# mozack/vdjer

Measured on AMD Instinct MI355X. Metric: M paired-reads/sec (k-mer build + contig score), IgH 50bp PE, higher is better.
Workload: dtype u8/u64 (2-bit packed bases, integer counts)

## Files before the change

### vdjer_amd/csrc/vdjx_score.hip

```cpp
#include "vdjx_common.h"
#include "vdjx_scan.h"

#include <algorithm>
#include <numeric>
#include <string.h>
#include <stdlib.h>
#include <stdio.h>

#define NONE32 0xFFFFFFFFu

__host__ __device__ inline int base_code(char ch) {
	const unsigned c = (unsigned char) ch;
	const int code = (int) ((0xD8u >> (((c >> 1) & 3u) * 2u)) & 3u);
	return (c == 'A' || c == 'C' || c == 'G' || c == 'T') ? code : -1;
}

extern "C" int vdjx_vregion_load(vdjx_ctx* c, const char* const* lines, size_t n_lines, int vk) {
	if (!c || (n_lines && !lines)) { vdjx_set_error("vdjx_vregion_load: NULL argument"); return VDJX_EINVAL; }
	if (vk < 2 || vk > 16) { vdjx_set_error("vregion k-mer size %d outside [2,16]", vk); return VDJX_ELIMIT; }
	HIP_TRY(hipSetDevice(c->device));
	vdjx_clear_errors();
	std::vector<u32> off(n_lines + 1, 0);
	std::string text;
	for (size_t i = 0; i < n_lines; i++) {
// ... 760 lines not shown
	auto drain = [&]() {
		vdjx_wave_lds_fence();
		for (u32 q0 = 0; q0 < qn; q0 += 64) {
			const u32 qi = q0 + (u32) lane;
			bool pr = false;
			u64 e = 0;
			u32 pos2 = 0, which = 0, o = 0;
			if (qi < qn) {
				e = q_ent[wv][qi]; o = q_off[wv][qi];
				pr = map_eval_entry(L, ix.rl, (int) o, e, pos2, which);
			}
			const u64 m = __ballot(pr);
			if (m) {
				u32 base = 0;
				if (lane == 0) base = atomicAdd(&pair_cnt[wi], (u32) __popcll(m));
				base = (u32) __builtin_amdgcn_readlane((int) base, 0);
				if (pr) {
					const u32 mult = ent_count(e);
					pairs[base + (u32) __popcll(m & ((1ull << lane) - 1ull))] = ((u64) mult << 32) | ((o + 1) << 16) | pos2;
					mine += mult;
				}
			}
		}
		vdjx_wave_lds_fence();
		qn = 0;
	};
	for (;;) {
		u32 hb = 0;
		if (lane == 0) hb = atomicAdd(&s_next, 64u * WP_K);
		hb = (u32) __builtin_amdgcn_readlane((int) hb, 0);
		if (hb >= h1) break;
		int orow = 0;
		{
			const u32 hr = hb + (u32) lane * 64u;
			if (lane < WP_K && hr < h1) {
				int lo = 0, hi = noff;
				while (hi - lo > 1) { const int mid = (lo + hi) >> 1; if (L.hpre[mid] <= hr) lo = mid; else hi = mid; }
				orow = lo;
			}
		}
		u64 ent[WP_K];
		u32 oo[WP_K / 2];
#pragma unroll
		for (int u = 0; u < WP_K; u++) {
			const u32 h = hb + (u32) (u * 64 + lane);
			int o = __builtin_amdgcn_readlane(orow, u);
			u64 e = ~0ull;
			if (h < h1) {
				while (h >= L.hpre[o + 1]) o++;
				e = ix.d8[L.cstart[o] + (h - L.hpre[o])];
			}
			ent[u] = e;
			if (u & 1) oo[u >> 1] |= (u32) o << 16; else oo[u >> 1] = (u32) o;
		}
#pragma unroll
		for (int u = 0; u < WP_K; u++) {
			if (hb + (u32) (u * 64) >= h1) break;
			const bool pass = map_entry_present(L, ent[u]) && hb + (u32) (u * 64 + lane) < h1;
			const u64 m = __ballot(pass);
			if (!m) continue;
			if (pass) {
				const u32 at = qn + (u32) __popcll(m & ((1ull << lane) - 1ull));
				q_ent[wv][at] = ent[u];
				q_off[wv][at] = (unsigned short) ((oo[u >> 1] >> (16 * (u & 1))) & 0xFFFFu);
			}
			qn += (u32) __popcll(m);
			if (qn > WP_Q - 64) drain();
		}
	}
	drain();
	mine = (u32) __builtin_amdgcn_readlane(vdjx_wave_scan_add((int) mine), 63);
	if (lane == 0 && mine) atomicAdd(&pair_np[wi], mine);
}

#define GP_G 8
#ifndef GP_THREADS
#define GP_THREADS 768
#define GP_WAVES 6
#define GP_K 12
#define GP_Q 128
#endif
#define GP_TS 4096u
#define GP_DMAX 2048u
#define GP_NOFF 512
#define GP_OCC (GP_G * GP_NOFF)
#define GP_PRESENT_LOG2 16
#ifndef GP_XCD_TILE
#define GP_XCD_TILE 1
#endif
static_assert(GP_Q >= 128, "a drain of full rows must find one");
struct GroupImg {
	u32 key[GP_TS];
	unsigned short didx[GP_TS];
	u32 hpre[GP_DMAX + 1];
	u32 cstart[GP_DMAX];
	unsigned short occ_start[GP_DMAX + 2];
	unsigned short wmask[GP_DMAX];
	unsigned short occ[GP_OCC];
	u32 present[1u << (GP_PRESENT_LOG2 - 5)];
};
__device__ inline int gp_lookup(const GroupImg& L, u32 cls) {
	u32 slot = cls & (GP_TS - 1);
	for (;;) {
		const u32 cur = L.key[slot];
		if (cur == 0) return -1;
		if (cur == cls + 1) return (int) L.didx[slot];
		slot = (slot + 1) & (GP_TS - 1);
	}
}
__device__ inline u32 gp_present_bit2(u32 cls) { return (cls * 0x9E3779B1u) >> (32 - GP_PRESENT_LOG2); }
__device__ inline bool gp_entry_present(const GroupImg& L, const u64 e) {
	const u32 ca = ent_a(e), cb = ent_b(e);
	const u32 ba = ca & ((1u << GP_PRESENT_LOG2) - 1u), bb = cb & ((1u << GP_PRESENT_LOG2) - 1u);
	const u32 ha = (L.present[ba >> 5] >> (ba & 31)) & 1u, hb = (L.present[bb >> 5] >> (bb & 31)) & 1u;
	if (!(ha | hb)) return false;
	const u32 ba2 = gp_present_bit2(ca), bb2 = gp_present_bit2(cb);
	return ((ha & (L.present[ba2 >> 5] >> (ba2 & 31))) | (hb & (L.present[bb2 >> 5] >> (bb2 & 31)))) & 1u;
}

__global__ __launch_bounds__(GP_THREADS, GP_WAVES) void k_group_pairs(ReadIndexDev ix, const uint4* __restrict__ prep, const u32* __restrict__ hits, u32 n, int len,
                                                              const u32* __restrict__ gorder, const u64* __restrict__ pair_off, u64* __restrict__ pair_buf,
                                                              u32* __restrict__ pair_cnt, u32* __restrict__ pair_np, u32* __restrict__ done, unsigned long long* __restrict__ gstat, u32 dbg_in,
                                                              u64 cap) {
#ifdef VDJX_ABLATE
	const u32 dbg = dbg_in;
#else
	(void) dbg_in;
	constexpr u32 dbg = 0u;
#endif
	if (pair_off[n] + 1 > cap) return;
	const long long t_begin = clock64();
	__shared__ GroupImg L;
	__shared__ u64 q_ent[GP_THREADS / 64][GP_Q];
	__shared__ unsigned short q_d[GP_THREADS / 64][GP_Q];
	__shared__ u64 s_pbase[GP_G];
	__shared__ u32 s_w[GP_G], s_pcnt[GP_G], s_np[GP_G], s_tmp[GP_THREADS / 64];
	__shared__ u32 s_nd, s_next, s_over;
	const int noff = len - ix.rl;
	const u32 tid = threadIdx.x;
	const int lane = __lane_id();
	const u32 wv = tid >> 6;
	u32 gblk = blockIdx.x;
#ifndef GP_XCD_M
#define GP_XCD_M 32u
#endif
	if (GP_XCD_TILE && (gblk | (8u * GP_XCD_M - 1u)) < gridDim.x) gblk = (gblk & ~(8u * GP_XCD_M - 1u)) | ((gblk & 7u) * GP_XCD_M) | ((gblk >> 3) & (GP_XCD_M - 1u));
	if (tid < GP_G) {
		const u32 idx = gblk * GP_G + tid;
		const u32 wi = idx < n ? gorder[idx] : NONE32;
		s_w[tid] = wi;
		s_pbase[tid] = wi != NONE32 ? pair_off[wi] : 0ull;
		s_pcnt[tid] = 0; s_np[tid] = 0;
	}
	if (tid == 0) { s_nd = 0; s_next = 0; s_over = 0; }
	for (u32 i = tid; i < GP_TS; i += GP_THREADS) L.key[i] = 0;
	for (u32 i = tid; i < (1u << (GP_PRESENT_LOG2 - 5)); i += GP_THREADS) L.present[i] = 0;
	__syncthreads();
	if (tid == 0) {
		u64 tot = 0;
		for (int w = 0; w < GP_G; w++) if (s_w[w] != NONE32) tot += hits[s_w[w]];
		if (tot >> 32) s_over = 1;
	}
	const u32 items = (u32) GP_G * (u32) noff;
	for (u32 it = tid; it < items; it += GP_THREADS) {
		const u32 w = it / (u32) noff, o = it - w * (u32) noff;
		if (s_w[w] == NONE32) continue;
		const uint4 p = prep[(size_t) s_w[w] * noff + o];
		const u32 cls = p.x;
		if (cls == NONE32) continue;
		const u32 pb = cls & ((1u << GP_PRESENT_LOG2) - 1u), pb2 = gp_present_bit2(cls);
		atomicOr(&L.present[pb >> 5], 1u << (pb & 31));
		atomicOr(&L.present[pb2 >> 5], 1u << (pb2 & 31));
		u32 slot = cls & (GP_TS - 1);
		for (u32 probes = 0;; probes++) {
			u32 cur = L.key[slot];
			if (cur == 0) {
				cur = atomicCAS(&L.key[slot], 0u, cls + 1);
				if (cur == 0) {
					const u32 d = atomicAdd(&s_nd, 1u);
					if (d < GP_DMAX) { L.didx[slot] = (unsigned short) d; L.cstart[d] = p.y; L.hpre[d] = p.z; }
					else s_over = 1;
					break;
				}
			}
			if (cur == cls + 1) break;
			slot = (slot + 1) & (GP_TS - 1);
			if (probes >= GP_TS) { s_over = 1; break; }
		}
	}
	__syncthreads();
	if (s_over) { if (tid == 0) atomicAdd(&gstat[1], 1ull); return; }
	const u32 nd = s_nd;
	u32* ocnt = (u32*) &q_ent[0][0];
	for (u32 i = tid; i < nd; i += GP_THREADS) ocnt[i] = 0;
	__syncthreads();
	for (u32 it = tid; it < items; it += GP_THREADS) {
		const u32 w = it / (u32) noff, o = it - w * (u32) noff;
		if (s_w[w] == NONE32) continue;
		const u32 cls = prep[(size_t) s_w[w] * noff + o].x;
		if (cls != NONE32) atomicAdd(&ocnt[gp_lookup(L, cls)], 1u);
	}
	__syncthreads();
	{
		constexpr u32 PER = (GP_DMAX + GP_THREADS) / GP_THREADS;
		u32 hv[PER], cv[PER], hs = 0, cs = 0;
#pragma unroll
		for (u32 j = 0; j < PER; j++) {
			const u32 a = PER * tid + j;
			hv[j] = a < nd ? L.hpre[a] : 0u; cv[j] = a < nd ? ocnt[a] : 0u;
			hs += hv[j]; cs += cv[j];
		}
		u32 htot, ctot;
		u32 hx = vdjx_block_scan(hs, s_tmp, htot);
		u32 cx = vdjx_block_scan(cs, s_tmp, ctot);
		__syncthreads();
#pragma unroll
		for (u32 j = 0; j < PER; j++) {
			const u32 a = PER * tid + j;
			if (a <= nd) { L.hpre[a] = hx; L.occ_start[a] = (unsigned short) cx; }
			if (a < nd) ocnt[a] = 0;
			hx += hv[j]; cx += cv[j];
		}
	}
	__syncthreads();
	for (int w = 0; w < GP_G; w++) {
		if (s_w[w] != NONE32)
			for (int o = (int) tid; o < noff; o += GP_THREADS) {
				const u32 cls = prep[(size_t) s_w[w] * noff + o].x;
				if (cls == NONE32) continue;
				const int d = gp_lookup(L, cls);
				L.occ[L.occ_start[d] + (atomicAdd(&ocnt[d], 1u) & 0xFFFFu)] = (unsigned short) ((u32) w << 10 | (u32) o);
				if (atomicOr(&ocnt[d], 0x10000u << w) & (0x10000u << w)) atomicOr(&ocnt[d], 0x80000000u);
			}
		__syncthreads();
	}
	for (u32 i = tid; i < nd; i += GP_THREADS) L.wmask[i] = (unsigned short) (ocnt[i] >> 16);
	__syncthreads();
	const u32 H = dbg == 2 ? 0u : L.hpre[nd];
	if (tid == 0) { atomicAdd(&gstat[0], (unsigned long long) H); atomicAdd(&gstat[2], (unsigned long long) nd); }
	u32 qn = 0, nq = 0;
	auto drain = [&](bool all) {
		vdjx_wave_lds_fence();
		const u32 upto = all ? qn : qn & ~63u;
		for (u32 q0 = 0; q0 < (dbg == 1 ? 0u : upto); q0 += 64) {
			const u32 qi = q0 + (u32) lane;
			if (qi >= qn) continue;
			const u64 e = q_ent[wv][qi];
			const u32 d = q_d[wv][qi];
			const u32 ca = ent_a(e), cb = ent_b(e);
			u32 as = 0, ae = 0, bs = 0, be = 0;
			int xa = -1, xb = -1;
			if (ca != RI_ENT_NONE) { xa = gp_lookup(L, ca); if (xa >= 0) { as = L.occ_start[xa]; ae = L.occ_start[xa + 1]; } }
			if (cb != RI_ENT_NONE) { xb = gp_lookup(L, cb); if (xb >= 0) { bs = L.occ_start[xb]; be = L.occ_start[xb + 1]; } }
			if (as == ae && bs == be) continue;
			const u32 fl = ent_flags(e), mult = ent_count(e);
			const u32 rc1 = (fl & RI_RC) ? 1u : 0u;
			const u32 mc = L.wmask[d], ma = as < ae ? (u32) L.wmask[xa] : 0u, mb = bs < be ? (u32) L.wmask[xb] : 0u;
			const u32 cs = L.occ_start[d];
			auto emit = [&](u32 w, u32 o, u32 la, u32 lb) {
				const u32 which = (lb && lb >= la) ? 1u : 0u;
				const u32 best = which ? lb : la;
				const u32 rc2 = (fl & (which ? RI_RCB : RI_RCA)) ? 1u : 0u;
				if (rc1 == rc2) return;
				const int dd = (int) (o + 1) - (int) best;
				const int insert = (int) (short) ((dd < 0 ? -dd : dd) + ix.rl);
				if (insert < 50 || insert > 400) return;
				const u32 pos = atomicAdd(&s_pcnt[w], 1u);
				pair_buf[s_pbase[w] + pos] = ((u64) mult << 32) | ((o + 1) << 16) | best;
				atomicAdd(&s_np[w], mult);
			};
			if (!((mc | ma | mb) & 0x8000u)) {
				for (u32 m = mc & (ma | mb); m; m &= m - 1) {
					const u32 w = (u32) __ffs((int) m) - 1u, below = (1u << w) - 1u;
					const u32 o = (u32) L.occ[cs + (u32) __popc(mc & below)] & 1023u;
					const u32 la = (ma >> w) & 1u ? ((u32) L.occ[as + (u32) __popc(ma & below)] & 1023u) + 1u : 0u;
					const u32 lb = (mb >> w) & 1u ? ((u32) L.occ[bs + (u32) __popc(mb & below)] & 1023u) + 1u : 0u;
					emit(w, o, la, lb);
				}
				continue;
			}
			u32 i = cs;
			const u32 ce = L.occ_start[d + 1];
			while (i < ce) {
				const u32 w = (u32) L.occ[i] >> 10;
				u32 la = 0, lb = 0;
				while (as < ae && ((u32) L.occ[as] >> 10) < w) as++;
				while (as < ae && ((u32) L.occ[as] >> 10) == w) { const u32 x = ((u32) L.occ[as] & 1023u) + 1u; la = x > la ? x : la; as++; }
				while (bs < be && ((u32) L.occ[bs] >> 10) < w) bs++;
				while (bs < be && ((u32) L.occ[bs] >> 10) == w) { const u32 x = ((u32) L.occ[bs] & 1023u) + 1u; lb = x > lb ? x : lb; bs++; }
				for (; i < ce && ((u32) L.occ[i] >> 10) == w; i++)
					if (la | lb) emit(w, (u32) L.occ[i] & 1023u, la, lb);
			}
		}
		const u32 rem = qn - upto;
		u64 me = 0; unsigned short md = 0;
		if ((u32) lane < rem) { me = q_ent[wv][upto + (u32) lane]; md = q_d[wv][upto + (u32) lane]; }
		vdjx_wave_lds_fence();
		if ((u32) lane < rem && upto) { q_ent[wv][lane] = me; q_d[wv][lane] = md; }
		vdjx_wave_lds_fence();
		qn = rem;
	};
	for (;;) {
		u32 hb = 0;
		if (lane == 0) hb = atomicAdd(&s_next, 64u * GP_K);
		hb = (u32) __builtin_amdgcn_readlane((int) hb, 0);
		if (hb >= H) break;
		int drow = 0;
		{
			const u32 hr = hb + (u32) lane * 64u;
			if (lane < GP_K && hr < H) {
				int lo = 0, hi = (int) nd;
				while (hi - lo > 1) { const int mid = (lo + hi) >> 1; if (L.hpre[mid] <= hr) lo = mid; else hi = mid; }
				drow = lo;
			}
		}
		u64 ent[GP_K];
		u32 dd[GP_K / 2];
#pragma unroll
		for (int u = 0; u < GP_K; u++) {
			const u32 h = hb + (u32) (u * 64 + lane);
			int d = __builtin_amdgcn_readlane(drow, u);
			u64 e = ~0ull;
			if (h < H) {
				while (h >= L.hpre[d + 1]) d++;
				e = ix.d8[L.cstart[d] + (h - L.hpre[d])];
			}
			ent[u] = e;
			if (u & 1) dd[u >> 1] |= (u32) d << 16; else dd[u >> 1] = (u32) d;
		}
#pragma unroll
		for (int u = 0; u < GP_K; u++) {
			if (hb + (u32) (u * 64) >= H) break;
			const bool pass = gp_entry_present(L, ent[u]) && hb + (u32) (u * 64 + lane) < H;
			const u64 m = __ballot(pass);
			if (!m) continue;
			if (pass) {
				const u32 at = qn + (u32) __popcll(m & ((1ull << lane) - 1ull));
				q_ent[wv][at] = ent[u];
				q_d[wv][at] = (unsigned short) ((dd[u >> 1] >> (16 * (u & 1))) & 0xFFFFu);
			}
			qn += (u32) __popcll(m); nq += (u32) __popcll(m);
			if (qn > GP_Q - 64) drain(false);
		}
	}
	drain(true);
	if (lane == 0 && nq) atomicAdd(&gstat[3], (unsigned long long) nq);
	__syncthreads();
	if (tid < GP_G && s_w[tid] != NONE32) { pair_cnt[s_w[tid]] = s_pcnt[tid]; pair_np[s_w[tid]] = s_np[tid]; done[s_w[tid]] = 1u; }
	if (tid == 0) {
		const unsigned long long dt = (unsigned long long) (clock64() - t_begin);
		atomicAdd(&gstat[4], dt);
		atomicMax(&gstat[5], dt);
	}
}

__global__ __launch_bounds__(MAP_THREADS) void k_window_cover(int len, int rl, vdjx_cov_params cp, const u32* __restrict__ order,
                                                              const u64* __restrict__ pair_off, const u64* __restrict__ pair_buf,
                                                              const u32* __restrict__ pair_cnt, uint8_t* __restrict__ out_valid,
                                                              u64* __restrict__ dbg) {
	const long long t_begin = dbg ? clock64() : 0;
	constexpr int HF_WORDS = MAP_MAXOFF + VDJX_MAX_READ_LEN + 2;
	static_assert(4 * ((HF_WORDS + COV_WORDS) * 4 + 3 * 4) <= 160 * 1024, "k_window_cover: 4 workgroups per CU need hf + diff + flags <= 40 KiB");
	__shared__ u32 hf[HF_WORDS];
	__shared__ int diff[COV_WORDS];
	__shared__ u32 s_bad, s_ok;
	__shared__ int s_firstv;
	const u32 tid = threadIdx.x;
	const int D = len + 1;
	const int e0 = cp.eval_start, e1 = cp.eval_stop, fl = cp.floor;
	const int gap = rl - cp.read_span;
	const int clo = cp.insert_low - rl - cp.mate_span / 2;
	const int chi = cp.insert_high - rl + cp.mate_span / 2;
	const int npos = e1 - e0;
	const int stride = npos + 1;
	const int DB = COV_WORDS / stride;
	const u32 wi = order[blockIdx.x];
	const u64* pairs = pair_buf + pair_off[wi];
	const u32 npairs = pair_cnt[wi];
	if (fl == 0) { if (tid == 0) out_valid[wi] = 1; return; }
	const u32 wv = tid >> 6, NW = MAP_THREADS / 64;
	u32* hp = (u32*) diff;
	const bool priv = (u32) (D + 1) * NW <= COV_WORDS;
	for (u32 i = tid; i < (u32) D + 1; i += MAP_THREADS) hf[i] = 0;
	if (priv) for (u32 i = tid; i < (u32) (D + 1) * NW; i += MAP_THREADS) hp[i] = 0;
	if (tid == 0) { s_bad = 0; s_ok = 0; }
	__syncthreads();
	u32* myh = priv ? hp + wv * (u32) (D + 1) : hf;
	for (u32 q = tid; q < npairs; q += MAP_THREADS) {
		const u64 pe = pairs[q];
		const u32 pr = (u32) pe, mult = (u32) (pe >> 32);
		atomicAdd(&myh[pr >> 16], mult);
		atomicAdd(&myh[pr & 0xFFFFu], mult);
	}
	__syncthreads();
	if (priv) {
		for (u32 i = tid; i < (u32) D + 1; i += MAP_THREADS) {
			u32 sum = 0;
			for (u32 w2 = 0; w2 < NW; w2++) sum += hp[w2 * (u32) (D + 1) + i];
			hf[i] = sum;
		}
		__syncthreads();
	}
	if (tid < 64) {
		const int per = (D + 63) / 64;
		const int a0 = (int) tid * per;
		const int b0 = a0 + per < D ? a0 + per : D;
		u32 sum = 0;
		for (int q = a0; q < b0; q++) sum += hf[q];
		const u32 incl = (u32) vdjx_wave_scan_add((int) sum);
		u32 run = incl - sum;
		for (int q = a0; q < b0; q++) { run += hf[q]; hf[q] = run; }
	}
	if (tid == 0) s_firstv = 0x7FFFFFFF;
	__syncthreads();
	{
		const int n_ent = (int) hf[D - 1];
		const int vmax = e1 - cp.read_span + 1;
		const int vlo = e0 > 1 ? e0 : 1;
		for (int v = vlo + (int) tid; v <= vmax && v < D; v += MAP_THREADS) {
			const int cv = (int) hf[v], cv1 = (int) hf[v - 1];
			if (cv == cv1) continue;
			atomicMin(&s_firstv, v);
			const int i0 = cv1;
			if (i0 < fl) s_bad = 1;
			const int pg = v - gap - 1;
// ... 356 lines not shown
	const int noff = len - ix.rl;
	char* d_s;
	u32 *d_hits, *d_inst;
	PlanOut* d_tot;
	HIP_TRY(db.alloc(&d_s, n * len));
	HIP_TRY(db.alloc(&mp->d_prep, n * (size_t) noff));
	HIP_TRY(db.alloc(&d_hits, n));
	HIP_TRY(db.alloc(&d_inst, n));
	HIP_TRY(db.alloc(&mp->d_off, n + 1));
	HIP_TRY(db.alloc(&mp->d_order, n));
	HIP_TRY(db.alloc(&mp->d_wstart, n + 1));
	HIP_TRY(db.alloc(&d_tot, 1));
	u64 *d_gkey = nullptr, *d_gkey2 = nullptr;
	u32* d_gidx = nullptr;
	if (grouped) {
		HIP_TRY(db.alloc(&d_gkey, n));
		HIP_TRY(db.alloc(&d_gkey2, n));
		HIP_TRY(db.alloc(&d_gidx, n));
		HIP_TRY(db.alloc(&mp->d_gorder, n));
	}
	mp->d_hits = d_hits;
	const char* d_src = nullptr;
	if (vdjx_host_block_holds(c, strings, n * (size_t) len)) d_src = strings;
	const u32 pieces = d_src ? 1u : n * (size_t) len >= (2u << 20) ? 4u : 1u;
	if (pieces > 1) {
		HIP_TRY(hipEventRecord(c->ev_up[0], st));
		HIP_TRY(hipStreamWaitEvent(c->up_stream, c->ev_up[0], 0));
	}
	for (u32 pc = 0; pc < pieces; pc++) {
		const size_t a = n * (size_t) pc / pieces, b = n * (size_t) (pc + 1) / pieces;
		if (pieces > 1) {
			HIP_TRY(hipMemcpyAsync(d_s + a * len, strings + a * len, (b - a) * len, hipMemcpyHostToDevice, c->up_stream));
			HIP_TRY(hipEventRecord(c->ev_up[1 + pc], c->up_stream));
			HIP_TRY(hipStreamWaitEvent(st, c->ev_up[1 + pc], 0));
		} else if (!d_src)
			HIP_TRY(hipMemcpyAsync(d_s, strings, n * len, hipMemcpyHostToDevice, st));
		vdjx_prof_scope ps(c, "k_map_classify");
		const dim3 grid((u32) std::min<size_t>(b - a, 8192));
		if (d_src) d_s = const_cast<char*>(d_src);
		if (c->ri_pool->W == 2) hipLaunchKernelGGL(k_map_classify<2>, grid, dim3(MAP_THREADS), 0, st, ix, d_s, (u32) b, len, weighted, mp->d_prep, d_hits, d_inst, d_gkey, d_gidx, (u32) a);
		else hipLaunchKernelGGL(k_map_classify<VDJX_LONG_W>, grid, dim3(MAP_THREADS), 0, st, ix, d_s, (u32) b, len, weighted, mp->d_prep, d_hits, d_inst, d_gkey, d_gidx, (u32) a);
	}
	{
		vdjx_prof_scope ps(c, "k_plan");
		const bool staged = n * 4 <= 96 * 1024;
		if (staged) HIP_TRY(hipFuncSetAttribute((const void*) k_plan, hipFuncAttributeMaxDynamicSharedMemorySize, 96 * 1024));
		hipLaunchKernelGGL(k_plan, dim3(1), dim3(1024), staged ? n * 4 : 0, st, d_hits, d_inst, (u32) n, chunk_fixed, weighted ? 1 : 0, weighted ? 1 : 0, mp->d_off, mp->d_order, mp->d_wstart, d_tot,
		                   staged ? 1 : 0);
	}
	if (grouped) {
		vdjx_prof_scope ps(c, "group_sort");
		const int rc = vdjx_sort_pairs(db, st, d_gkey, d_gkey2, d_gidx, mp->d_gorder, (u32) n, 22);
		if (rc) return rc;
	}
	HIP_TRY(c->h_plan.reserve(256, 0));
	HIP_TRY(hipMemcpyAsync(c->h_plan, d_tot, sizeof(PlanOut), hipMemcpyDeviceToHost, st));
	HIP_TRY(hipEventRecord(c->ev_plan, st));
	lp.mark("plan_issue");
	return wait ? plan_finish(c, mp) : VDJX_OK;
}

__global__ void k_gather_u64(const u64* __restrict__ src, const u64* __restrict__ move, u64* __restrict__ dst) {
	const u64 so = move[3 * (size_t) blockIdx.x], dof = move[3 * (size_t) blockIdx.x + 1], cnt = move[3 * (size_t) blockIdx.x + 2];
	for (u64 i = threadIdx.x; i < cnt; i += blockDim.x) dst[dof + i] = src[so + i];
}

static int cov_params_check(const vdjx_cov_params* p, const char* who) {
	if (p->eval_start < 1 || p->eval_stop <= p->eval_start) { vdjx_set_error("%s: bad eval range", who); return VDJX_EINVAL; }
	if (p->eval_stop - p->eval_start + 1 > COV_WORDS) { vdjx_set_error("%s: eval range too long", who); return VDJX_ELIMIT; }
	return VDJX_OK;
}

static int window_pairs_run(vdjx_ctx* c, vdjx_work& db, const ReadIndexDev& ix, const char* windows, size_t n, int len, u32** d_np_out,
                            u32** d_cnt_out, MapPlan* mp, u64 budget = 0, u64* need = nullptr) {
	hipStream_t st = c->stream;
	u32 *d_np, *d_cnt;
	static const u32 hit_chunk = (u32) vdjx_env_num("VDJX_HIT_CHUNK", HIT_CHUNK, 1, 0xFFFFFFFFll);
	static const bool group_on = vdjx_env_num("VDJX_WINDOW_GROUP", 1, 0, 1) != 0;
#ifdef VDJX_ABLATE
	static const u32 gp_dbg = (u32) vdjx_env_num("VDJX_GP_DBG", 0, 0, 2);
#else
	constexpr u32 gp_dbg = 0;
#endif
	static const size_t group_min = (size_t) vdjx_env_num("VDJX_GROUP_MIN", 4096, 0, 1ll << 40);
	const bool grouped = group_on && len - ix.rl <= GP_NOFF && n >= group_min;
	constexpr u32 left_chunk = 32768u;
	int rc = classify_and_plan(c, db, ix, windows, n, len, true, grouped && left_chunk < hit_chunk ? left_chunk : hit_chunk, mp, grouped, false);
	if (rc) return rc;
	const size_t nq = (n + 3) & ~(size_t) 3;
	u32* d_zero;
	HIP_TRY(db.alloc(&d_zero, (grouped ? 3 : 2) * nq + (grouped ? 16 : 0)));
	d_np = d_zero; d_cnt = d_zero + nq;
	u32* d_done = nullptr;
	unsigned long long* d_gstat = nullptr;
	if (grouped) { d_done = d_zero + 2 * nq; d_gstat = (unsigned long long*) (d_zero + 3 * nq); }
	auto map_groups = [&]() -> int {
		HIP_TRY(hipMemsetAsync(d_zero, 0, ((grouped ? 3 : 2) * nq + (grouped ? 16 : 0)) * 4, st));
		if (!grouped) return VDJX_OK;
		vdjx_prof_scope ps(c, "k_group_pairs");
		hipLaunchKernelGGL(k_group_pairs, dim3((u32) ((n + GP_G - 1) / GP_G)), dim3(GP_THREADS), 0, st, ix, mp->d_prep, mp->d_hits, (u32) n, len, mp->d_gorder,
		                   mp->d_off, (u64*) c->wp_buf, d_cnt, d_np, d_done, d_gstat, gp_dbg, (u64) (c->wp_buf.bytes / 8));
		return VDJX_OK;
	};
	const bool early = grouped && c->wp_buf.bytes > 0;
	if (early && (rc = map_groups())) return rc;
	if ((rc = plan_finish(c, mp))) return rc;
	const u64 total = mp->tot.total_hits;
	bool again = !early;
	if (need) *need = 0;
	const size_t wp_need = ((size_t) total + 1) * 8;
	if (wp_need > c->wp_buf.bytes && budget && n > 1 && (total + total / 4 + 1024) * 8 > budget) {
		HIP_TRY(hipStreamSynchronize(st));
		*need = (total + total / 4 + 1024) * 8;
		return VDJX_OK;
	}
	if (wp_need > c->wp_buf.bytes) {
		HIP_TRY(hipStreamSynchronize(st));
		HIP_TRY(c->wp_buf.reserve(wp_need, ((size_t) total / 4 + 1023) * 8));
		again = true;
	}
	if (again && (rc = map_groups())) return rc;
	c->stats["window_hits"] = mp->tot.inst_total;
	c->stats["window_hits_max"] = mp->tot.inst_max;
	c->stats["window_hits_distinct"] = total;
	c->stats["window_work_items"] = mp->tot.nwork;
	if (mp->tot.nwork) {
		u32* d_witem = nullptr;
		if (grouped) HIP_TRY(db.alloc(&d_witem, (size_t) mp->tot.nwork + 1));
		vdjx_prof_scope ps(c, "k_window_pairs");
		if (grouped) hipLaunchKernelGGL(k_work_items, dim3((u32) (n / 256 + 1)), dim3(256), 0, st, mp->d_wstart, (u32) n, d_witem);
		if (len - ix.rl <= 512)
			hipLaunchKernelGGL(k_window_pairs<512>, dim3(mp->tot.nwork), dim3(MAP_THREADS), 0, st, ix, mp->d_prep, (u32) n, len, mp->tot.chunk, mp->d_order, mp->d_wstart,
			                   mp->d_off, (u64*) c->wp_buf, d_cnt, d_np, d_done, d_gstat ? d_gstat + 1 : nullptr, (const u32*) d_witem);
		else
			hipLaunchKernelGGL(k_window_pairs<MAP_MAXOFF>, dim3(mp->tot.nwork), dim3(MAP_THREADS), 0, st, ix, mp->d_prep, (u32) n, len, mp->tot.chunk, mp->d_order, mp->d_wstart,
			                   mp->d_off, (u64*) c->wp_buf, d_cnt, d_np, d_done, d_gstat ? d_gstat + 1 : nullptr, (const u32*) d_witem);
	}
	if (d_gstat) HIP_TRY(hipMemcpyAsync((char*) c->h_plan + 128, d_gstat, 64, hipMemcpyDeviceToHost, st));
	mp->gstat = d_gstat != nullptr;
	*d_np_out = d_np; *d_cnt_out = d_cnt;
	return VDJX_OK;
}

static int window_score_slice(vdjx_ctx* c, const ReadIndexDev& ix, const char* windows, size_t n, int len, const vdjx_cov_params* p,
                              uint8_t* out_valid, uint32_t* out_npairs, u64 budget, u64* need) {
	hipStream_t st = c->stream;
	vdjx_work db(c);
	u32 *d_np, *d_cnt;
	uint8_t* d_valid;
	MapPlan mp;
	HIP_TRY(db.alloc(&d_valid, n));
	int rc = window_pairs_run(c, db, ix, windows, n, len, &d_np, &d_cnt, &mp, budget, need);
	if (rc || *need) return rc;
	c->wp_n = 0;
	{
		vdjx_prof_scope ps(c, "k_window_cover");
		u64* d_clk = nullptr;
		static const bool cover_clocks = vdjx_env_set("VDJX_COVER_CLOCKS");
		if (cover_clocks) HIP_TRY(db.alloc(&d_clk, n));
		hipLaunchKernelGGL(k_window_cover, dim3((u32) n), dim3(MAP_THREADS), 0, st, len, ix.rl, *p, mp.d_order, mp.d_off, (const u64*) c->wp_buf, d_cnt, d_valid, d_clk);
		if (cover_clocks) {
			std::vector<u64> clk(n);
			std::vector<u32> cnt(n), ord(n);
			std::vector<uint8_t> val(n);
			HIP_TRY(hipStreamSynchronize(st));
			HIP_TRY(hipMemcpy(clk.data(), d_clk, n * 8, hipMemcpyDeviceToHost));
			HIP_TRY(hipMemcpy(cnt.data(), d_cnt, n * 4, hipMemcpyDeviceToHost));
			HIP_TRY(hipMemcpy(ord.data(), mp.d_order, n * 4, hipMemcpyDeviceToHost));
			HIP_TRY(hipMemcpy(val.data(), d_valid, n, hipMemcpyDeviceToHost));
			std::vector<u32> by(n);
			for (size_t i = 0; i < n; i++) by[i] = (u32) i;
			std::sort(by.begin(), by.end(), [&](u32 a, u32 b) { return clk[a] > clk[b]; });
			u64 sum = 0;
			for (size_t i = 0; i < n; i++) sum += clk[i];
			fprintf(stderr, "cover clocks: %zu windows, sum %llu, slowest:", n, (unsigned long long) sum);
			for (size_t i = 0; i < n && i < 8; i++) {
				size_t at = 0;
				while (at < n && ord[at] != by[i]) at++;
				fprintf(stderr, " [w%u blk%zu entries %u valid %d clk %llu]", by[i], at, cnt[by[i]], (int) val[by[i]], (unsigned long long) clk[by[i]]);
			}
			fprintf(stderr, "\n");
		}
	}
	const size_t nres = ((n + 15) & ~(size_t) 15) + 8 * n;
	HIP_TRY(c->h_res.reserve(nres, nres / 4));
	uint8_t* hr_valid = (uint8_t*) c->h_res;
	u32* hr_np = (u32*) (hr_valid + ((n + 15) & ~(size_t) 15));
	u32* hr_cnt = hr_np + n;
	HIP_TRY(hipMemcpyAsync(hr_valid, d_valid, n, hipMemcpyDeviceToHost, st));
	HIP_TRY(hipMemcpyAsync(hr_np, d_np, n * 4, hipMemcpyDeviceToHost, st));
	HIP_TRY(hipMemcpyAsync(hr_cnt, d_cnt, n * 4, hipMemcpyDeviceToHost, st));
	vdjx_laps lp(c);
	HIP_TRY(hipStreamSynchronize(st));
	HIP_TRY(hipGetLastError());
	lp.mark("ws_cover_wait");
	memcpy(out_valid, hr_valid, n);
	memcpy(out_npairs, hr_np, n * 4);
	c->wp_cnt.assign(hr_cnt, hr_cnt + n);
	vdjx_prof_collect(c, false);
	if (mp.gstat) {
		const unsigned long long* g = (const unsigned long long*) ((const char*) c->h_plan + 128);
		c->stats["group_hits_distinct"] = g[0];
		c->stats["group_overflows"] = g[1];
		c->stats["group_classes"] = g[2];
		c->stats["group_queued"] = g[3];
		c->stats["group_clocks_sum"] = g[4];
		c->stats["group_clocks_max"] = g[5];
	}
	{
		u64 tot = 0, ent = 0;
		for (size_t i = 0; i < n; i++) { tot += out_npairs[i]; ent += c->wp_cnt[i]; }
		c->stats["window_pairs"] = tot;
		c->stats["window_pairs_entries"] = ent;
	}
	return VDJX_OK;
}

extern "C" int vdjx_window_score(vdjx_ctx* c, const char* windows, size_t n, int len, const vdjx_cov_params* p,
                                 uint8_t* out_valid, uint32_t* out_npairs) {
	if (!c || !p || (n && (!windows || !out_valid || !out_npairs))) { vdjx_set_error("vdjx_window_score: NULL argument"); return VDJX_EINVAL; }
	if (n == 0) return VDJX_OK;
	ReadIndexDev ix;
	int rc = make_index_view(c, &ix, len, "vdjx_window_score");
	if (rc) return rc;
	if ((rc = cov_params_check(p, "vdjx_window_score"))) return rc;
	if (n >= (1ull << 31)) { vdjx_set_error("vdjx_window_score: too many windows"); return VDJX_ELIMIT; }
	HIP_TRY(hipSetDevice(c->device));
	vdjx_clear_errors();
	static const u64 budget_env = (u64) vdjx_env_num("VDJX_WP_BUDGET_MB", 0, 0, 1ll << 40) << 20;
	u64 budget = budget_env;
	if (!budget) {
		size_t fr = 0, tt = 0;
		HIP_TRY(hipMemGetInfo(&fr, &tt));
		budget = ((u64) fr + (u64) c->wp_buf.bytes) / 10 * 8;
	}
	static const char* const summed[] = {"window_hits", "window_hits_distinct", "window_work_items", "group_hits_distinct", "group_overflows", "group_classes",
	                                     "group_queued", "window_pairs", "window_pairs_entries"};
	std::map<std::string, uint64_t> acc;
	u64 hits_max = 0, slices = 0;
	size_t at = 0, step = n;
	while (at < n) {
		const size_t m = std::min(step, n - at);
		u64 need = 0;
		rc = window_score_slice(c, ix, windows + at * (size_t) len, m, len, p, out_valid + at, out_npairs + at, budget, &need);
		if (rc) return rc;
		if (need) {
			step = std::max<size_t>(1, std::min<size_t>(m - 1, (size_t) ((double) m * (double) budget / (double) need * 0.8)));
			continue;
		}
		for (const char* k_ : summed) acc[k_] += c->stats[k_];
		hits_max = std::max<u64>(hits_max, c->stats["window_hits_max"]);
		slices++;
		at += m;
	}
	if (slices > 1) {
		for (const char* k_ : summed) c->stats[k_] = acc[k_];
		c->stats["window_hits_max"] = hits_max;
	}
	c->stats["window_slices"] = slices;
	return VDJX_OK;
}

extern "C" int vdjx_window_pairs(vdjx_ctx* c, const char* windows, size_t n, int len, uint32_t* out_entries, uint32_t* out_npairs) {
	if (!c || (n && (!windows || !out_entries || !out_npairs))) { vdjx_set_error("vdjx_window_pairs: NULL argument"); return VDJX_EINVAL; }
	if (c) c->wp_n = 0;
	if (n == 0) return VDJX_OK;
	ReadIndexDev ix;
	int rc = make_index_view(c, &ix, len, "vdjx_window_pairs");
	if (rc) return rc;
	if (n >= (1ull << 31)) { vdjx_set_error("vdjx_window_pairs: too many windows"); return VDJX_ELIMIT; }
	HIP_TRY(hipSetDevice(c->device));
	vdjx_clear_errors();
	hipStream_t st = c->stream;
	vdjx_work db(c);
	u32 *d_np, *d_cnt;
	MapPlan mp;
	rc = window_pairs_run(c, db, ix, windows, n, len, &d_np, &d_cnt, &mp);
	if (rc) return rc;
	c->wp_cnt.resize(n);
	c->wp_off.resize(n + 1);
	HIP_TRY(hipMemcpyAsync(c->wp_cnt.data(), d_cnt, n * 4, hipMemcpyDeviceToHost, st));
	HIP_TRY(hipMemcpyAsync(c->wp_off.data(), mp.d_off, (n + 1) * 8, hipMemcpyDeviceToHost, st));
	HIP_TRY(hipMemcpyAsync(out_npairs, d_np, n * 4, hipMemcpyDeviceToHost, st));
	HIP_TRY(hipStreamSynchronize(st));
	HIP_TRY(hipGetLastError());
	vdjx_prof_collect(c, false);
	memcpy(out_entries, c->wp_cnt.data(), n * 4);
	c->wp_n = n;
	return VDJX_OK;
}
// ... 552 lines not shown
```

Baseline: 965.4.

## Scan big hit classes as full 64-entry rows and queue entry indices

Classes with at least 64 hit entries are now split into full 64-wide rows that are handed out to waves in batches. Each lane reads one entry of a row, which gives coalesced loads and avoids the per-lane class search used for the tail. The per-wave queue now stores 32-bit entry indices instead of 64-bit entries, and the drain re-reads each entry from global memory, trading LDS space for an extra load. The emit path is also changed to wave-wide ballots, so all lanes share one atomic slot reservation per step, at the cost of more divergent control flow and added complexity.

```diff
diff --git a/vdjer_amd/csrc/vdjx_score.hip b/vdjer_amd/csrc/vdjx_score.hip
--- a/vdjer_amd/csrc/vdjx_score.hip
+++ b/vdjer_amd/csrc/vdjx_score.hip
@@ -866,6 +866,7 @@
 #endif
 #define GP_TS 4096u
 #define GP_DMAX 2048u
+#define GP_BIG 1024u
 #define GP_NOFF 512
 #define GP_OCC (GP_G * GP_NOFF)
 #define GP_PRESENT_LOG2 16
@@ -877,7 +878,9 @@
 	u32 key[GP_TS];
 	unsigned short didx[GP_TS];
 	u32 hpre[GP_DMAX + 1];
-	u32 cstart[GP_DMAX];
+	u32 tbase[GP_DMAX];
+	u32 rpre[GP_BIG + 1];
+	unsigned short rcls[GP_BIG];
 	unsigned short occ_start[GP_DMAX + 2];
 	unsigned short wmask[GP_DMAX];
 	unsigned short occ[GP_OCC];
@@ -905,7 +908,7 @@
 __global__ __launch_bounds__(GP_THREADS, GP_WAVES) void k_group_pairs(ReadIndexDev ix, const uint4* __restrict__ prep, const u32* __restrict__ hits, u32 n, int len,
                                                               const u32* __restrict__ gorder, const u64* __restrict__ pair_off, u64* __restrict__ pair_buf,
                                                               u32* __restrict__ pair_cnt, u32* __restrict__ pair_np, u32* __restrict__ done, unsigned long long* __restrict__ gstat, u32 dbg_in,
-                                                              u64 cap) {
+                                                              u64 cap, u32 big_max) {
 #ifdef VDJX_ABLATE
 	const u32 dbg = dbg_in;
 #else
@@ -915,11 +918,11 @@
 	if (pair_off[n] + 1 > cap) return;
 	const long long t_begin = clock64();
 	__shared__ GroupImg L;
-	__shared__ u64 q_ent[GP_THREADS / 64][GP_Q];
-	__shared__ unsigned short q_d[GP_THREADS / 64][GP_Q];
+	__shared__ struct { u32 idx[GP_THREADS / 64][GP_Q]; unsigned short d[GP_THREADS / 64][GP_Q]; } Q;
 	__shared__ u64 s_pbase[GP_G];
 	__shared__ u32 s_w[GP_G], s_pcnt[GP_G], s_np[GP_G], s_tmp[GP_THREADS / 64];
-	__shared__ u32 s_nd, s_next, s_over;
+	__shared__ u32 s_nd, s_next, s_nextr, s_over;
+	static_assert(sizeof(Q) >= GP_DMAX * sizeof(u32), "the occurrence counters of the image build lie in the idle queues");
 	const int noff = len - ix.rl;
 	const u32 tid = threadIdx.x;
 	const int lane = __lane_id();
@@ -936,7 +939,7 @@
 		s_pbase[tid] = wi != NONE32 ? pair_off[wi] : 0ull;
 		s_pcnt[tid] = 0; s_np[tid] = 0;
 	}
-	if (tid == 0) { s_nd = 0; s_next = 0; s_over = 0; }
+	if (tid == 0) { s_nd = 0; s_next = 0; s_nextr = 0; s_over = 0; }
 	for (u32 i = tid; i < GP_TS; i += GP_THREADS) L.key[i] = 0;
 	for (u32 i = tid; i < (1u << (GP_PRESENT_LOG2 - 5)); i += GP_THREADS) L.present[i] = 0;
 	__syncthreads();
@@ -962,7 +965,7 @@
 				cur = atomicCAS(&L.key[slot], 0u, cls + 1);
 				if (cur == 0) {
 					const u32 d = atomicAdd(&s_nd, 1u);
-					if (d < GP_DMAX) { L.didx[slot] = (unsigned short) d; L.cstart[d] = p.y; L.hpre[d] = p.z; }
+					if (d < GP_DMAX) { L.didx[slot] = (unsigned short) d; L.tbase[d] = p.y; L.hpre[d] = p.z; }
 					else s_over = 1;
 					break;
 				}
@@ -975,7 +978,7 @@
 	__syncthreads();
 	if (s_over) { if (tid == 0) atomicAdd(&gstat[1], 1ull); return; }
 	const u32 nd = s_nd;
-	u32* ocnt = (u32*) &q_ent[0][0];
+	u32* ocnt = (u32*) &Q;
 	for (u32 i = tid; i < nd; i += GP_THREADS) ocnt[i] = 0;
 	__syncthreads();
 	for (u32 it = tid; it < items; it += GP_THREADS) {
@@ -985,26 +988,43 @@
 		if (cls != NONE32) atomicAdd(&ocnt[gp_lookup(L, cls)], 1u);
 	}
 	__syncthreads();
+	u32 nbig;
 	{
 		constexpr u32 PER = (GP_DMAX + GP_THREADS) / GP_THREADS;
-		u32 hv[PER], cv[PER], hs = 0, cs = 0;
+		u32 hv[PER], cv[PER], fv[PER], cs = 0, hs = 0, fs = 0;
 #pragma unroll
 		for (u32 j = 0; j < PER; j++) {
 			const u32 a = PER * tid + j;
 			hv[j] = a < nd ? L.hpre[a] : 0u; cv[j] = a < nd ? ocnt[a] : 0u;
-			hs += hv[j]; cs += cv[j];
-		}
-		u32 htot, ctot;
+			cs += cv[j] + (hv[j] >= 64u ? 0x10000u : 0u);
+		}
+		u32 ctot, htot, ftot;
+		u32 cx = vdjx_block_scan(cs, s_tmp, ctot);
+		u32 bx = cx >> 16, full = 0;
+#pragma unroll
+		for (u32 j = 0; j < PER; j++) {
+			if (hv[j] >= 64u) full |= 1u << j;
+			fv[j] = hv[j] >= 64u && bx < big_max ? hv[j] >> 6 : 0u;
+			bx += (full >> j) & 1u;
+			hv[j] -= 64u * fv[j];
+			hs += hv[j]; fs += fv[j];
+		}
 		u32 hx = vdjx_block_scan(hs, s_tmp, htot);
-		u32 cx = vdjx_block_scan(cs, s_tmp, ctot);
+		u32 fx = vdjx_block_scan(fs, s_tmp, ftot);
+		nbig = (u32) __builtin_amdgcn_readfirstlane((int) ((ctot >> 16) < big_max ? ctot >> 16 : big_max));
+		bx = cx >> 16;
+		cx &= 0xFFFFu;
 		__syncthreads();
 #pragma unroll
 		for (u32 j = 0; j < PER; j++) {
 			const u32 a = PER * tid + j;
 			if (a <= nd) { L.hpre[a] = hx; L.occ_start[a] = (unsigned short) cx; }
-			if (a < nd) ocnt[a] = 0;
-			hx += hv[j]; cx += cv[j];
-		}
+			if (a < nd) { ocnt[a] = 0; L.tbase[a] += 64u * fv[j] - hx; }
+			if (fv[j]) { L.rpre[bx] = fx; L.rcls[bx] = (unsigned short) a; }
+			bx += (full >> j) & 1u;
+			hx += hv[j]; cx += cv[j]; fx += fv[j];
+		}
+		if (tid == 0) L.rpre[nbig] = ftot;
 	}
 	__syncthreads();
 	for (int w = 0; w < GP_G; w++) {
@@ -1021,69 +1041,145 @@
 	for (u32 i = tid; i < nd; i += GP_THREADS) L.wmask[i] = (unsigned short) (ocnt[i] >> 16);
 	__syncthreads();
 	const u32 H = dbg == 2 ? 0u : L.hpre[nd];
-	if (tid == 0) { atomicAdd(&gstat[0], (unsigned long long) H); atomicAdd(&gstat[2], (unsigned long long) nd); }
+	const u32 R = dbg == 2 ? 0u : (u32) __builtin_amdgcn_readfirstlane((int) L.rpre[nbig]);
+	if (tid == 0) {
+		atomicAdd(&gstat[0], (unsigned long long) H + 64ull * R); atomicAdd(&gstat[2], (unsigned long long) nd);
+		atomicAdd(&gstat[6], 64ull * R);
+	}
+	const u64 lt = (1ull << lane) - 1ull;
 	u32 qn = 0, nq = 0;
-	auto drain = [&](bool all) {
+	auto drain = [&](bool all) __attribute__((always_inline)) {
 		vdjx_wave_lds_fence();
 		const u32 upto = all ? qn : qn & ~63u;
 		for (u32 q0 = 0; q0 < (dbg == 1 ? 0u : upto); q0 += 64) {
 			const u32 qi = q0 + (u32) lane;
-			if (qi >= qn) continue;
-			const u64 e = q_ent[wv][qi];
-			const u32 d = q_d[wv][qi];
+			bool live = qi < qn;
+			u64 e = 0;
+			u32 d = 0;
+			if (live) { e = ix.d8[Q.idx[wv][qi]]; d = Q.d[wv][qi]; }
 			const u32 ca = ent_a(e), cb = ent_b(e);
 			u32 as = 0, ae = 0, bs = 0, be = 0;
 			int xa = -1, xb = -1;
-			if (ca != RI_ENT_NONE) { xa = gp_lookup(L, ca); if (xa >= 0) { as = L.occ_start[xa]; ae = L.occ_start[xa + 1]; } }
-			if (cb != RI_ENT_NONE) { xb = gp_lookup(L, cb); if (xb >= 0) { bs = L.occ_start[xb]; be = L.occ_start[xb + 1]; } }
-			if (as == ae && bs == be) continue;
+			if (live && ca != RI_ENT_NONE) { xa = gp_lookup(L, ca); if (xa >= 0) { as = L.occ_start[xa]; ae = L.occ_start[xa + 1]; } }
+			if (live && cb != RI_ENT_NONE) { xb = gp_lookup(L, cb); if (xb >= 0) { bs = L.occ_start[xb]; be = L.occ_start[xb + 1]; } }
+			live = live && !(as == ae && bs == be);
 			const u32 fl = ent_flags(e), mult = ent_count(e);
 			const u32 rc1 = (fl & RI_RC) ? 1u : 0u;
-			const u32 mc = L.wmask[d], ma = as < ae ? (u32) L.wmask[xa] : 0u, mb = bs < be ? (u32) L.wmask[xb] : 0u;
+			const u32 mc = live ? (u32) L.wmask[d] : 0u, ma = as < ae ? (u32) L.wmask[xa] : 0u, mb = bs < be ? (u32) L.wmask[xb] : 0u;
 			const u32 cs = L.occ_start[d];
-			auto emit = [&](u32 w, u32 o, u32 la, u32 lb) {
+			auto emit = [&](u32 w, bool on, u32 o, u32 la, u32 lb) {
 				const u32 which = (lb && lb >= la) ? 1u : 0u;
 				const u32 best = which ? lb : la;
 				const u32 rc2 = (fl & (which ? RI_RCB : RI_RCA)) ? 1u : 0u;
-				if (rc1 == rc2) return;
 				const int dd = (int) (o + 1) - (int) best;
 				const int insert = (int) (short) ((dd < 0 ? -dd : dd) + ix.rl);
-				if (insert < 50 || insert > 400) return;
-				const u32 pos = atomicAdd(&s_pcnt[w], 1u);
-				pair_buf[s_pbase[w] + pos] = ((u64) mult << 32) | ((o + 1) << 16) | best;
-				atomicAdd(&s_np[w], mult);
+				const bool em = on && rc1 != rc2 && !(insert < 50 || insert > 400);
+				const u64 m = __ballot(em);
+				if (!m) return;
+				u32 pos = 0;
+				if (lane == 0) pos = atomicAdd(&s_pcnt[w], (u32) __popcll(m));
+				pos = (u32) __builtin_amdgcn_readlane((int) pos, 0) + (u32) __popcll(m & lt);
+				if (em) pair_buf[s_pbase[w] + pos] = ((u64) mult << 32) | ((o + 1) << 16) | best;
+				const u32 sum = (u32) __builtin_amdgcn_readlane(vdjx_wave_scan_add((int) (em ? mult : 0u)), 63);
+				if (lane == 0) atomicAdd(&s_np[w], sum);
 			};
-			if (!((mc | ma | mb) & 0x8000u)) {
-				for (u32 m = mc & (ma | mb); m; m &= m - 1) {
-					const u32 w = (u32) __ffs((int) m) - 1u, below = (1u << w) - 1u;
-					const u32 o = (u32) L.occ[cs + (u32) __popc(mc & below)] & 1023u;
-					const u32 la = (ma >> w) & 1u ? ((u32) L.occ[as + (u32) __popc(ma & below)] & 1023u) + 1u : 0u;
-					const u32 lb = (mb >> w) & 1u ? ((u32) L.occ[bs + (u32) __popc(mb & below)] & 1023u) + 1u : 0u;
-					emit(w, o, la, lb);
+			const bool rep = ((mc | ma | mb) & 0x8000u) != 0u;
+			const u32 once = rep ? 0u : mc & (ma | mb);
+			for (u32 w = 0; w < GP_G; w++) {
+				const bool on = (once >> w) & 1u;
+				if (!__ballot(on)) continue;
+				u32 o = 0, la = 0, lb = 0;
+				if (on) {
+					const u32 under = (1u << w) - 1u;
+					o = (u32) L.occ[cs + (u32) __popc(mc & under)] & 1023u;
+					la = (ma >> w) & 1u ? ((u32) L.occ[as + (u32) __popc(ma & under)] & 1023u) + 1u : 0u;
+					lb = (mb >> w) & 1u ? ((u32) L.occ[bs + (u32) __popc(mb & under)] & 1023u) + 1u : 0u;
 				}
-				continue;
-			}
+				emit(w, on, o, la, lb);
+			}
+			if (!__ballot(rep)) continue;
 			u32 i = cs;
-			const u32 ce = L.occ_start[d + 1];
-			while (i < ce) {
-				const u32 w = (u32) L.occ[i] >> 10;
+			const u32 ce = rep ? (u32) L.occ_start[d + 1] : cs;
+			for (u32 w = 0; w < GP_G; w++) {
 				u32 la = 0, lb = 0;
-				while (as < ae && ((u32) L.occ[as] >> 10) < w) as++;
-				while (as < ae && ((u32) L.occ[as] >> 10) == w) { const u32 x = ((u32) L.occ[as] & 1023u) + 1u; la = x > la ? x : la; as++; }
-				while (bs < be && ((u32) L.occ[bs] >> 10) < w) bs++;
-				while (bs < be && ((u32) L.occ[bs] >> 10) == w) { const u32 x = ((u32) L.occ[bs] & 1023u) + 1u; lb = x > lb ? x : lb; bs++; }
-				for (; i < ce && ((u32) L.occ[i] >> 10) == w; i++)
-					if (la | lb) emit(w, (u32) L.occ[i] & 1023u, la, lb);
+				if (rep) {
+					while (as < ae && ((u32) L.occ[as] >> 10) < w) as++;
+					while (as < ae && ((u32) L.occ[as] >> 10) == w) { const u32 x = ((u32) L.occ[as] & 1023u) + 1u; la = x > la ? x : la; as++; }
+					while (bs < be && ((u32) L.occ[bs] >> 10) < w) bs++;
+					while (bs < be && ((u32) L.occ[bs] >> 10) == w) { const u32 x = ((u32) L.occ[bs] & 1023u) + 1u; lb = x > lb ? x : lb; bs++; }
+				}
+				for (;;) {
+					const bool has = i < ce && ((u32) L.occ[i] >> 10) == w;
+					if (!__ballot(has)) break;
+					u32 o = 0;
+					if (has) { o = (u32) L.occ[i] & 1023u; i++; }
+					emit(w, has && (la | lb), o, la, lb);
+				}
 			}
 		}
 		const u32 rem = qn - upto;
-		u64 me = 0; unsigned short md = 0;
-		if ((u32) lane < rem) { me = q_ent[wv][upto + (u32) lane]; md = q_d[wv][upto + (u32) lane]; }
+		u32 me = 0; unsigned short md = 0;
+		if ((u32) lane < rem) { me = Q.idx[wv][upto + (u32) lane]; md = Q.d[wv][upto + (u32) lane]; }
 		vdjx_wave_lds_fence();
-		if ((u32) lane < rem && upto) { q_ent[wv][lane] = me; q_d[wv][lane] = md; }
+		if ((u32) lane < rem && upto) { Q.idx[wv][lane] = me; Q.d[wv][lane] = md; }
 		vdjx_wave_lds_fence();
 		qn = rem;
 	};
+	auto push = [&](bool pass, auto idx, u32 d) __attribute__((always_inline)) {
+		const u64 m = __ballot(pass);
+		if (!m) return;
+		if (pass) {
+			const u32 at = qn + (u32) __popcll(m & lt);
+			Q.idx[wv][at] = idx();
+			Q.d[wv][at] = (unsigned short) d;
+		}
+		qn += (u32) __popcll(m); nq += (u32) __popcll(m);
+		if (qn > GP_Q - 64) drain(false);
+	};
+	for (;;) {
+		u32 rb = 0;
+		if (lane == 0) rb = atomicAdd(&s_nextr, (u32) GP_K);
+		rb = (u32) __builtin_amdgcn_readlane((int) rb, 0);
+		if (rb >= R) break;
+		u32 rbase = 0, rd = 0;
+		if (lane < GP_K) {
+			const u32 r = rb + (u32) lane < R ? rb + (u32) lane : rb;
+			int lo = 0, hi = (int) nbig;
+			while (hi - lo > 1) { const int mid = (lo + hi) >> 1; if (L.rpre[mid] <= r) lo = mid; else hi = mid; }
+			rd = L.rcls[lo];
+			rbase = L.tbase[rd] + L.hpre[rd] + 64u * (r - L.rpre[lo + 1]);
+		}
+		u64 ent[GP_K];
+#pragma unroll
+		for (int u = 0; u < GP_K; u++) {
+			const u64* row = ix.d8 + (u32) __builtin_amdgcn_readlane((int) rbase, u);
+			ent[u] = row[lane];
+		}
+		u32 pm = 0;
+#pragma unroll
+		for (int u = 0; u < GP_K; u++) pm |= gp_entry_present(L, ent[u]) ? 1u << u : 0u;
+		if (R - rb < (u32) GP_K) pm &= (1u << (R - rb)) - 1u;
+		const u32 cnt = (u32) __popc(pm), incl = (u32) vdjx_wave_scan_add((int) cnt);
+		const u32 total = (u32) __builtin_amdgcn_readlane((int) incl, 63);
+		if (total == 0) continue;
+		if (qn + total <= GP_Q) {
+			u32 at = qn + incl - cnt;
+			for (u32 left = pm; __ballot(left != 0u);) {
+				const u32 u = left ? (u32) __ffs((int) left) - 1u : 0u;
+				const u32 b = (u32) __shfl((int) rbase, (int) u, 64), d = (u32) __shfl((int) rd, (int) u, 64);
+				if (left) { Q.idx[wv][at] = b + (u32) lane; Q.d[wv][at] = (unsigned short) d; at++; left &= left - 1u; }
+			}
+			qn += total; nq += total;
+			if (qn > GP_Q - 64) drain(false);
+			continue;
+		}
+#pragma unroll 1
+		for (int u = 0; u < GP_K; u++) {
+			if (rb + (u32) u >= R) break;
+			const u32 b = (u32) __builtin_amdgcn_readlane((int) rbase, u);
+			push((pm >> u) & 1u, [&] { return b + (u32) lane; }, (u32) __builtin_amdgcn_readlane((int) rd, u));
+		}
+	}
 	for (;;) {
 		u32 hb = 0;
 		if (lane == 0) hb = atomicAdd(&s_next, 64u * GP_K);
@@ -1107,24 +1203,22 @@
 			u64 e = ~0ull;
 			if (h < H) {
 				while (h >= L.hpre[d + 1]) d++;
-				e = ix.d8[L.cstart[d] + (h - L.hpre[d])];
+				e = ix.d8[L.tbase[d] + h];
 			}
 			ent[u] = e;
 			if (u & 1) dd[u >> 1] |= (u32) d << 16; else dd[u >> 1] = (u32) d;
 		}
+		u32 pm = 0;
 #pragma unroll
+		for (int u = 0; u < GP_K; u++) pm |= gp_entry_present(L, ent[u]) && hb + (u32) (u * 64 + lane) < H ? 1u << u : 0u;
+#pragma unroll 1
 		for (int u = 0; u < GP_K; u++) {
 			if (hb + (u32) (u * 64) >= H) break;
-			const bool pass = gp_entry_present(L, ent[u]) && hb + (u32) (u * 64 + lane) < H;
-			const u64 m = __ballot(pass);
-			if (!m) continue;
-			if (pass) {
-				const u32 at = qn + (u32) __popcll(m & ((1ull << lane) - 1ull));
-				q_ent[wv][at] = ent[u];
-				q_d[wv][at] = (unsigned short) ((dd[u >> 1] >> (16 * (u & 1))) & 0xFFFFu);
-			}
-			qn += (u32) __popcll(m); nq += (u32) __popcll(m);
-			if (qn > GP_Q - 64) drain(false);
+			u32 d2 = dd[0];
+#pragma unroll
+			for (int v = 1; v < GP_K / 2; v++) d2 = (u >> 1) == v ? dd[v] : d2;
+			const u32 h = hb + (u32) (u * 64 + lane), d = (d2 >> (16 * (u & 1))) & 0xFFFFu;
+			push((pm >> u) & 1u, [&] { return L.tbase[d] + h; }, d);
 		}
 	}
 	drain(true);
@@ -1647,6 +1741,7 @@
 #else
 	constexpr u32 gp_dbg = 0;
 #endif
+	static const u32 gp_big_max = (u32) vdjx_env_num("VDJX_GP_BIG_MAX", GP_BIG, 0, GP_BIG);
 	static const size_t group_min = (size_t) vdjx_env_num("VDJX_GROUP_MIN", 4096, 0, 1ll << 40);
 	const bool grouped = group_on && len - ix.rl <= GP_NOFF && n >= group_min;
 	constexpr u32 left_chunk = 32768u;
@@ -1664,7 +1759,7 @@
 		if (!grouped) return VDJX_OK;
 		vdjx_prof_scope ps(c, "k_group_pairs");
 		hipLaunchKernelGGL(k_group_pairs, dim3((u32) ((n + GP_G - 1) / GP_G)), dim3(GP_THREADS), 0, st, ix, mp->d_prep, mp->d_hits, (u32) n, len, mp->d_gorder,
-		                   mp->d_off, (u64*) c->wp_buf, d_cnt, d_np, d_done, d_gstat, gp_dbg, (u64) (c->wp_buf.bytes / 8));
+		                   mp->d_off, (u64*) c->wp_buf, d_cnt, d_np, d_done, d_gstat, gp_dbg, (u64) (c->wp_buf.bytes / 8), gp_big_max);
 		return VDJX_OK;
 	};
 	const bool early = grouped && c->wp_buf.bytes > 0;
@@ -1771,6 +1866,7 @@
 		c->stats["group_queued"] = g[3];
 		c->stats["group_clocks_sum"] = g[4];
 		c->stats["group_clocks_max"] = g[5];
+		c->stats["group_hits_rows"] = g[6];
 	}
 	{
 		u64 tot = 0, ent = 0;
```

New measurement: 939.9. 2.6% lower.
